# noce2/FluidFramework

Hardware: AMD Instinct MI355X
Metric: sequenced merge-tree ops applied/sec (node) at 100k docs; bit-exact text+props (higher is better)
Workload: dtype int32; 1 GPU; c3: 100000 docs/GPU x 10000 sequenced ops, 8 writers, refSeq lag <= 64, insert 0.5 / remove 0.3 / annotate 0.2; docs_total=100000, docs_per_gpu=100000, ops_per_doc=10000, parallelism=doc-shard x1

## Files before the change

fluidframework_amd/__init__.py:

```python
import ctypes

import numpy as np

from . import _native
from .wire import CHECKSUM_DTYPE, OP_DTYPE, Batch, Interner

__all__ = ["MergeTreeBatch", "DeviceBatch", "Batch", "Interner", "DeltaLogOverflow"]


class DeltaLogOverflow(RuntimeError):

    def __init__(self, msg, records):
        super().__init__(msg)
        self.records = records


class PinnedArray:

    def __init__(self, lib, n, dtype):
        dt = np.dtype(dtype)
        nbytes = max(int(n), 1) * dt.itemsize
        self.lib = lib
        self.p = lib.mt_host_alloc(nbytes)
        if not self.p:
# ... 347 lines not shown
        if not b:
            raise RuntimeError(f"mt_generate failed: {self.lib.mt_last_error(self.h).decode()}")
        return DeviceBatch(self, None, handle=b)

    def generated_seeds(self, cfg, doc_base=0, doc_ids=None):
        c = _native.gen_cfg(cfg)
        ids = None if doc_ids is None else np.ascontiguousarray(doc_ids, dtype=np.int32)
        off = np.zeros(self.n_docs + 1, dtype=np.int64)
        self._check(self.lib.mt_generated_seeds_docs(self.h, ctypes.byref(c), doc_base, _native.ptr(ids),
                                                     _native.ptr(off), None), "mt_generated_seeds")
        seed = np.zeros(max(int(off[-1]), 1), dtype=np.uint16)
        self._check(self.lib.mt_generated_seeds_docs(self.h, ctypes.byref(c), doc_base, _native.ptr(ids),
                                                     _native.ptr(off), _native.ptr(seed)), "mt_generated_seeds")
        return off, seed

    def sync(self):
        self._check(self.lib.mt_sync(self.h), "mt_sync")

    def last_hbm_docs(self):
        out = np.zeros(8, dtype=np.uint32)
        self._check(self.lib.mt_last_hbm_docs(self.h, _native.ptr(out)), "mt_last_hbm_docs")
        return dict(total=int(out[0]), spilled=int(out[1]), segments=int(out[2]), blocks=int(out[3]), heap=int(out[4]),
                    text=int(out[5]), props=int(out[6]), at_load=int(out[7]))

    def last_paged_peaks(self):
        out = np.zeros(5, dtype=np.uint32)
        self._check(self.lib.mt_last_paged_peaks(self.h, _native.ptr(out)), "mt_last_paged_peaks")
        return dict(pages=int(out[0]), unsettled=int(out[1]), heap=int(out[2]), segments=int(out[3]),
                    tight_handovers=int(out[4]))

    def last_zamboni(self):
        out = np.zeros(2, dtype=np.uint32)
        self._check(self.lib.mt_last_zamboni(self.h, _native.ptr(out)), "mt_last_zamboni")
        return {"in_place": int(out[0]), "fallback": int(out[1])}

    def last_grown(self):
        out = np.zeros(6, dtype=np.uint32)
        self._check(self.lib.mt_last_grown(self.h, _native.ptr(out)), "mt_last_grown")
        return dict(zip(["grown", "rounds", "in_big_region", "pages", "unsettled", "heap"], (int(x) for x in out)))

    def last_kernel_ms(self):
        return float(self.lib.mt_last_kernel_ms(self.h))

    def set_stream_priority(self, priority):
        self._check(self.lib.mt_set_stream_priority(self.h, int(priority)), "mt_set_stream_priority")

    def last_load_ms(self):
        return float(self.lib.mt_last_load_ms(self.h))

    def status(self):
        out = np.zeros(self.n_docs, dtype=np.int32)
        self._check(self.lib.mt_get_status(self.h, _native.ptr(out)), "mt_get_status")
        return out

    def get_length(self, doc):
        out = ctypes.c_uint32()
        self._check(self.lib.mt_get_length(self.h, doc, ctypes.byref(out)), "mt_get_length")
        return out.value

    def get_text(self, doc):
        n = ctypes.c_uint32()
        self._check(self.lib.mt_get_text(self.h, doc, None, 0, ctypes.byref(n)), "mt_get_text")
        buf = np.zeros(max(n.value, 1), dtype=np.uint16)
        self._check(self.lib.mt_get_text(self.h, doc, _native.ptr(buf), n.value, ctypes.byref(n)),
                    "mt_get_text")
        return buf[: n.value].tobytes().decode("utf-16-le", errors="surrogatepass")

# ... 282 lines not shown
```

fluidframework_amd/_native.py:

```python
import ctypes
import os

import numpy as np

from .wire import CHECKSUM_DTYPE, OP_DTYPE

HERE = os.path.dirname(os.path.abspath(__file__))
MT_E_INVALID, MT_E_HIP, MT_E_NOMEM, MT_E_NODEVICE, MT_E_OVERFLOW, MT_E_STALE_VIEW = -1, -2, -3, -4, -5, -6
LIB_PATH = os.environ.get("MT_LIB_PATH") or os.path.join(HERE, "libmtreplay.so")


class MtOptions(ctypes.Structure):
    _fields_ = [("device", ctypes.c_int32), ("seg_capacity", ctypes.c_int32),
                ("block_capacity", ctypes.c_int32), ("heap_capacity", ctypes.c_int32),
                ("text_capacity", ctypes.c_int32), ("props_capacity", ctypes.c_int32),
                ("delta_log_capacity", ctypes.c_int32), ("lds_seg_capacity", ctypes.c_int32),
                ("page_capacity", ctypes.c_int32), ("page_heap_capacity", ctypes.c_int32),
                ("unsettled_capacity", ctypes.c_int32), ("uid_capacity", ctypes.c_int32),
                ("lds_page_capacity", ctypes.c_int32), ("lds_unsettled_capacity", ctypes.c_int32),
                ("lds_page_heap_capacity", ctypes.c_int32), ("lds_narrow_overlap", ctypes.c_int32),
                ("delta_log_mode", ctypes.c_int32), ("live_client", ctypes.c_int32),
                ("live_group_capacity", ctypes.c_int32), ("paged_slices", ctypes.c_int32),
                ("segment_ordinals", ctypes.c_int32), ("overlap_arena_capacity", ctypes.c_int32)]

# ... 19 lines not shown
                ("p_newline", ctypes.c_uint64), ("p_len_continue", ctypes.c_uint64),
                ("p_insert_props", ctypes.c_uint64), ("p_null", ctypes.c_uint64)]


_P, _I, _U32, _U64 = ctypes.c_void_p, ctypes.c_int, ctypes.c_uint32, ctypes.c_uint64
SIGNATURES = [
    ("mt_create", _P, [_U32, _P]),
    ("mt_destroy", None, [_P]),
    ("mt_last_error", ctypes.c_char_p, [_P]),
    ("mt_num_docs", _U32, [_P]),
    ("mt_load_initial_text", _I, [_P, _P, _P]),
    ("mt_start_collaboration", _I, [_P, _P, _P]),
    ("mt_reset", _I, [_P]),
    ("mt_apply_ops", _I, [_P, _P, _P, _U64, _P, _U64, _P, _U64]),
    ("mt_load_snapshots", _I, [_P, _P, _P, _P, _U64, _P, _U64, _P, _U64, _P, _P]),
    ("mt_extract_snapshots", _I, [_P, _P, _P, _P, _P, _P, _P]),
    ("mt_snapshots_upload", _P, [_P, _P, _P, _P, _U64, _P, _U64, _P, _U64, _P, _P]),
    ("mt_snapshots_upload_range", _P, [_P, _U32, _U32, _P, _P, _P, _U64, _P, _U64, _P, _U64, _P, _P]),
    ("mt_snapshots_load_async", _I, [_P, _P]),
    ("mt_snapshots_free", None, [_P]),
    ("mt_batch_upload", _P, [_P, _P, _P, _U64, _P, _U64, _P, _U64]),
    ("mt_batch_apply_async", _I, [_P, _P]),
    ("mt_batch_num_ops", _U64, [_P]),
    ("mt_batch_free", None, [_P]),
    ("mt_host_alloc", ctypes.c_void_p, [ctypes.c_uint64]),
    ("mt_host_free", None, [ctypes.c_void_p]),
    ("mt_sync", _I, [_P]),
    ("mt_last_kernel_ms", ctypes.c_float, [_P]),
    ("mt_set_stream_priority", ctypes.c_int, [_P, ctypes.c_int]),
    ("mt_last_load_ms", ctypes.c_float, [_P]),
    ("mt_last_hbm_docs", _I, [_P, _P]),
    ("mt_last_paged_peaks", _I, [_P, _P]),
    ("mt_last_zamboni", _I, [_P, _P]),
    ("mt_last_grown", _I, [_P, _P]),
    ("mt_generate", _P, [_P, _P, _U32, _P]),
    ("mt_generate_docs", _P, [_P, _P, _U32, _P, _P, _P]),
    ("mt_generated_seeds_docs", _I, [_P, _P, _U32, _P, _P, _P]),
    ("mt_generated_seeds", _I, [_P, _P, _U32, _P, _P]),
    ("mt_batch_sizes", _I, [_P, _P, _P, _P]),
    ("mt_batch_download", _I, [_P, _P, _P, _P, _P]),
    ("mt_get_status", _I, [_P, _P]),
    ("mt_get_length", _I, [_P, _U32, _P]),
    ("mt_get_text", _I, [_P, _U32, _P, _U32, _P]),
    ("mt_get_texts", _I, [_P, _U32, _P, _P, _P, ctypes.c_uint16, _P, _P, _U64]),
    ("mt_get_texts_device", _I, [_P, _U32, _P, _P, _P, ctypes.c_uint16, _P, _P, _U64]),
    ("mt_last_text_ms", _I, [_P, _P]),
    ("mt_get_prop_runs", _I, [_P, _U32, _P, _U32, _P, _P, _U32, _P]),
    ("mt_get_segments", _I, [_P, _U32, _P, _U32, _P, _P, _U32, _P]),
    ("mt_get_segment_props", _I, [_P, _U32, _U32, _P, _U32, _P]),
    ("mt_get_all_segment_props", _I, [_P, _U32, _P, ctypes.c_uint64, _P]),
    ("mt_get_overlap_arena", _I, [_P, _U32, _P]),
    ("mt_get_delta_log", _I, [_P, _U32, _P, _U32, _P]),
    ("mt_delta_log_reset", _I, [_P]),
    ("mt_debug_raw", _I, [_P, _U32, _P, _U32, _P, _P]),
    ("mt_debug_prof", _I, [_P, _P, _I]),
    ("mt_maintenance_counts", _I, [_P, _P]),
    ("mt_checksums", _I, [_P, _P]),
    ("mt_checksums_device", _I, [_P, _P]),
    ("mt_regenerate_pending", _I, [_P, _U32, _P, _U32, _P, _P, _U32, _P, _U32]),
    ("mt_pending_counts", _I, [_P, _P]),
    ("mt_debug_heap", _I, [_P, _U32, _P, _U32, _P, _P, _U32, _P]),
    ("mt_get_containing_segment", _I, [_P, _U32, ctypes.c_int32, ctypes.c_int32, ctypes.c_int32, _P, _P, _U32]),
    ("mt_get_segment_by_uid", _I, [_P, _U32, _U32, ctypes.c_int32, ctypes.c_int32, _P, _P, _U32]),
    ("mt_get_view_lengths", _I, [_P, _U32, _P, _P, _P, _P]),
]

# ... 31 lines not shown
```

fluidframework_amd/csrc/mt_engine.h:

```cpp
#pragma once
#include <type_traits>

#include "mt_device.h"

#define LDS_AS __attribute__((address_space(3)))
#define GLB_AS __attribute__((address_space(1)))

template <bool kLogT> struct TierLdsT {
    static constexpr bool kLds = true;
    static constexpr bool kLog = kLogT;
    static constexpr bool kPaged = false;
    static constexpr bool kLive = false;
    static constexpr int kOvlBits = 32;
    static constexpr bool kMayGrow = false;
    static constexpr bool kOvf = false;
    typedef uint32_t O_v;
    typedef LDS_AS v4i *A_t;
    typedef LDS_AS uint32_t *O_t;
    typedef LDS_AS v4u *B_t;
    typedef LDS_AS v2i *H_t;
};
template <bool kLogT> struct TierGlbT {
    static constexpr bool kLds = false;
    static constexpr bool kLog = kLogT;
// ... 742 lines not shown
        wsync<T>();
        if (!has_parent) {
            const int nl = d.depth;
            if (nl >= MT_LV) {
                fail_cap(d, 2);
                return;
            }
            d.depth++;
            if (lane() == 0) {
                d.nb[nl] = 1;
                lvl(d, nl)[0] = 2;
            }
            wsync<T>();
            if (ordon(d)) ord_canon_all(d);
            return;
        }
        const int pc = cntr(d, l + 1, P) + 1;
        wsync<T>();
        if (lane() == 0) lvl(d, l + 1)[P] = (uint8_t)pc;
        wsync<T>();
        if (pc < MT_MAXN) {
            if (ordon(d)) {
                ord_put(ordl(d, l) + b + 1, uni((int)ordl(d, l)[b]) + ord_w(pc));
                ord_canon(d, l, b);
                ord_canon(d, l, b + 1);
            }
            return;
        }
        l = l + 1;
        b = P;
    }
}

TD void blk_replace(DocT<T> &d, int l, int b0, int nold, int k, int base, int extra) {
    if (nbr(d, l) + (k - nold) > bcap(d, l)) {
        fail_cap(d, 2);
        return;
    }
    blk_shift(d, l, b0 + nold, k - nold);
    LDS_AS uint8_t *c = lvl(d, l);
    for (int j = lane(); j < k; j += MT_WAVE) {
        c[b0 + j] = (uint8_t)(base + (j < extra ? 1 : 0));
        if (l == 0) d.flg[b0 + j] = MT_SCOUR_UNDEF;
    }
    wsync<T>();
}

TD void compute_ends(DocT<T> &d) {
    const LDS_AS uint8_t *c = lvl(d, 0);
    const int nb = nbr(d, 0);
    int carry = 0;
    for (int base = 0; base < nb; base += MT_WAVE) {
        const int b = base + lane();
        const int v = b < nb ? c[b] : 0;
        const int inc = wave_scan_incl(v);
        if (b < nb) d.ends[b] = (uint16_t)(carry + inc);
        carry += bcast(inc, MT_WAVE - 1);
    }
    wsync<T>();
}
TD int block_of(DocT<T> &d, int i, int nb) {
    int lo = 0, hi = nb - 1;
    while (lo < hi) {
        const int mid = (lo + hi) >> 1;
        if (d.ends[mid] > i)
            hi = mid;
// ... 1065 lines not shown
        }
        wsync<T>();
    }
    return keep;
}

#ifdef MT_PROF
TD void pack_impl(DocT<T> &d, int l, int b);
TD void pack(DocT<T> &d, int l, int b) {
    PROF_WRAP_BEGIN
    pack_impl(d, l, b);
    PROF_WRAP_END(3)
    
}
TD void pack_impl(DocT<T> &d, int l, int b) {
#else
TD void pack(DocT<T> &d, int l, int b) {
#endif
    while (true) {
        int c0;
        const int P = blk_find(d, l + 1, b, true, c0);
        if (P < 0) {
            FAIL_INTERNAL(d);
            return;
        }
        const int nch = cntr(d, l + 1, P);
        int total = 0;
        if (l == 0) {
            total = scour_range(d, blk_prefix(d, 0, c0), c0, nch);
            if (d.status) return;
        } else {
            for (int cb = c0; cb < c0 + nch; cb++) total += cntr(d, l, cb);
        }
        int k = total / MT_HALF;
        if (k > MT_MAXN - 1) k = MT_MAXN - 1;
        if (k < 1) k = 1;
        const int base = total / k, extra = total % k;
        blk_replace(d, l, c0, nch, k, base, extra);
        if (d.status) return;
        if (lane() == 0) lvl(d, l + 1)[P] = (uint8_t)k;
        wsync<T>();
        if (k < MT_HALF && l + 2 < d.depth) {
            l = l + 1;
            b = P;
            continue;
        }
        if (ordon(d)) ord_canon(d, l + 1, P);
        return;
    }
}

TD void pack_counts(DocT<T> &d, int l, int b, int &top_l, int &top_b) {
    while (true) {
        int c0;
        const int P = blk_find(d, l + 1, b, true, c0);
        if (P < 0) {
            FAIL_INTERNAL(d);
            return;
        }
        const int nch = cntr(d, l + 1, P);
        int total = 0;
        for (int cb = c0; cb < c0 + nch; cb++) total += cntr(d, l, cb);
        int k = total / MT_HALF;
        if (k > MT_MAXN - 1) k = MT_MAXN - 1;
        if (k < 1) k = 1;
        blk_replace(d, l, c0, nch, k, total / k, total % k);
        if (d.status) return;
        if (lane() == 0) lvl(d, l + 1)[P] = (uint8_t)k;
        wsync<T>();
        if (k < MT_HALF && l + 2 < d.depth) {
            l = l + 1;
            b = P;
            continue;
        }
        top_l = l + 1;
        top_b = P;
        return;
    }
}

#ifdef MT_PROF
TD void zamboni_impl(DocT<T> &d);
TD void zamboni(DocT<T> &d) {
    PROF_WRAP_BEGIN
    zamboni_impl(d);
    PROF_WRAP_END(4)
    
}
TD void zamboni_impl(DocT<T> &d) {
#else
TD void zamboni(DocT<T> &d) {
#endif
    for (int it = 0; it < MT_ZAMBONI && d.status == 0; it++) {
        if (d.heap_n == 0) break;
        const v2i top = heap_top(d);
        if (top.x > d.min_seq) break;
        heap_pop(d);
        wsync<T>();
        P2_T0(12)
// ... 879 lines not shown
```

fluidframework_amd/csrc/mt_kernels.h:

```cpp
#pragma once
#include "../../include/mt_replay.h"
#include "mt_paged.h"

__device__ static void init_doc_hdr(const DevState &st, int doc, int len) {
    DocHdr h;
    memset(&h, 0, sizeof(h));
    h.depth = 1;
    h.n_blk[0] = 1;
    h.text_top = len;
    h.props_top = 1;
    h.next_uid = 2;
    h.delta_hash = MT_FNV_OFF;
    h.status = len > st.T ? MT_DOC_CAPACITY : 0;
    const size_t S = st.S;
    if (len > 0) {
        h.n_seg = 1;
        st.segA[doc * S] = v4i{len, 0, MT_RSEQ_NONE, pack_cli(-1, 0)};
        st.segO[doc * S] = 0ull;
        st.segB[doc * S] = v4u{0u, 0u, 1u, 0u};
        if (st.segP) {
            u64 *w = (u64 *)(st.segP + doc * S);
            w[0] = w[1] = w[2] = w[3] = 0ull;
        }
    }
// ... 378 lines not shown
            q[0] = len;
            q[1] = d.n;
            q[2] = r;
            q[3] = c;
        }
        OpIn in;
        gen_op(g, cfg, t, r, c, msn, len, in, ops_out, text_out, props_out, doc);
        apply_op(d, in, gt, gp);
    }
    gen_end(g, used_out, doc);
    if (T::kLds && d.status == MT_DOC_RETRY) {
        if (lane() == 0) st.retry[doc] = 1;
        return;
    }
    if (lane() == 0) {
        if (d.status) fail_out[doc] = d.status;
        if (!T::kLds) st.retry[doc] = 0;
    }
    store_doc(d, st, doc);
}

template <class T>
__device__ __forceinline__ void pg_peaks(const DevState &st, PagedDoc<T> &pd, int pk_ut, int pk_heap) {
    const int np = nbr(pd.up, 1);
    int ns = 0;
    for (int q = lane(); q < np; q += MT_WAVE) ns += pm_nseg(pd, pd.up.dir[q]);
    ns = wave_sum(ns);
    if (lane() == 0) {
        atomicMax(st.stats + 8, (uint32_t)np);
        atomicMax(st.stats + 9, (uint32_t)pk_ut);
        atomicMax(st.stats + 10, (uint32_t)pk_heap);
        atomicMax(st.stats + 11, (uint32_t)ns);
        if constexpr (pg_zinplace<T>()) {
            const uint32_t zi = pg_zcount(pd)[0], zf = pg_zcount(pd)[1];
            if (zi) atomicAdd(st.stats + 16, zi);
            if (zf) atomicAdd(st.stats + 17, zf);
        }
    }
}
#ifndef MT_PAGED_WAVES
#define MT_PAGED_WAVES 3
#endif
#ifndef MT_HM_WAVES
#define MT_HM_WAVES 2
#endif
#ifndef MT_FULL_WAVES
#define MT_FULL_WAVES 2
#endif
#ifndef MT_PACKED_WAVES
#define MT_PACKED_WAVES 2
#endif
template <class T> constexpr int paged_waves() {
    return T::kHM ? MT_HM_WAVES
                  : (T::kMayGrow ? MT_FULL_WAVES : (T::kPacked ? MT_PACKED_WAVES : MT_PAGED_WAVES));
}
#if MT_PAGED_WAVES > 0
#define MT_PAGED_WPE __attribute__((amdgpu_waves_per_eu(paged_waves<T>())))
#else
#define MT_PAGED_WPE
#endif
template <class T>
__device__ __forceinline__ void pg_handover(const DevState &st, int doc, int64_t k, const PagedCaps &pc) {
    if (lane() == 0) {
        st.retry[doc] = pc.tight ? 2 : 3;
        st.resume[doc] = k;
        atomicAdd(st.stats + (pc.tight ? 12 : 13), 1u);
    }
}
struct PagedSlice {
// ... 240 lines not shown
```

fluidframework_amd/csrc/mt_paged.h:

```cpp
#pragma once
#include "mt_engine.h"

#ifdef MT_PROF
#define PG_T0(k) const unsigned long long _pt##k = __builtin_amdgcn_s_memtime();
#define PG_T1(k)                                                         \
    if (lane() == 0) {                                                   \
        pd.w.prof[k] += __builtin_amdgcn_s_memtime() - _pt##k;           \
        pd.w.prof[64 + k] += 1ull;                                       \
    }
#define PG_CNT(k)                                                        \
    if (lane() == 0) pd.w.prof[64 + k] += 1ull;
#else
#define PG_T0(k)
#define PG_T1(k)
#define PG_CNT(k)
#endif

template <class T> struct PagedDoc {
    DocT<T> w;
    DocT<T> up;
    LDS_AS PageMeta *meta;
    GLB_AS PageMeta *gmeta;
    LDS_AS int *pvl;
    LDS_AS int *cob;
// ... 33 lines not shown
    LDS_AS int *sob;
    int sob_ch;
    int wnb, wobs;
};

struct PagedCaps {
    int PP, PH, UT;
    int tight;
    int stage;
    int narrow;
    int grow;
    int packed;
};

#define PW_B 16
#define MT_PK_MASKS 256

struct PagedLayout {
    uint32_t offWA, offWB, offWO, offWcnt, offWflg, offWends, offWscr, offWnb;
    uint32_t offUcnt, offUnb, offDir, offMeta, offCob, offHeap, offUpage, offUA, offUO, offGen, offProf,
        total;
};
static __host__ __device__ inline PagedLayout paged_layout(int PP, int PH, int UT, int gen_words, int ob,
                                                           bool packed = false, bool hm = false) {
    PagedLayout L;
    uint32_t o = 0;
    L.offWA = o; o += 16u * MT_PG_SLOTS;
    L.offWB = o; o += 16u * MT_PG_SLOTS;
    L.offWO = o; o += (uint32_t)ob * MT_PG_SLOTS;
    L.offUA = o; o += (packed ? 12u : 16u) * UT;
    o = (o + 7u) & ~7u;
    L.offUO = o; o += packed ? 8u * MT_PK_MASKS + MT_PK_MASKS / 8 : ((((uint32_t)ob * UT) + 7u) & ~7u);
    L.offHeap = o; o += 8u * (PH + 1);
    L.offMeta = o; o += hm ? 0u : (uint32_t)sizeof(PageMeta) * PP + 8u;
    L.offUpage = o; o += packed ? 0u : (2u * UT + 3u) & ~3u;
    L.offCob = o; o += hm ? 8u * (uint32_t)((PP + 63) / 64) + 4u * 64 : 4u * PP;
    L.offWscr = o; o += 64u * 4;
    L.offWnb = o; o += MT_LV * 4;
    L.offUnb = o; o += MT_LV * 4;
    L.offGen = o; o += 4u * gen_words;
    L.offDir = o; o += 2u * PP;
    L.offWends = o; o += 2u * PW_B;
    L.offWcnt = o; o += (uint32_t)MT_LV * PW_B;
    L.offWflg = o; o += PW_B;
    L.offUcnt = o; o += (uint32_t)(pcnt_bytes(PP) - PP);
#ifdef MT_PROF
    o = (o + 7u) & ~7u;
    L.offProf = o; o += 128u * 8;
#else
    L.offProf = 0;
#endif
    L.total = (o + 15u) & ~15u;
    return L;
}

TD PagedDoc<T> &pdoc(DocT<T> &w) { return *reinterpret_cast<PagedDoc<T> *>(&w); }
template <class T> __device__ __forceinline__ PagedCaps eff_caps(PagedCaps pc) {
    if constexpr (T::kPP > 0) pc.PP = T::kPP;
    if constexpr (T::kPH > 0) pc.PH = T::kPH;
    if constexpr (T::kUT > 0) pc.UT = T::kUT;
    return pc;
}
TD void pg_fail_cap(DocT<T> &w, int cause) {
    if (w.status == 0) w.cap_cause = cause;
    fail(w, MT_DOC_CAPACITY);
}
__device__ __forceinline__ PageMeta pm_load(const LDS_AS PageMeta *m) {
// ... 981 lines not shown
        asm volatile("" ::"v"(touch));
#else
        pg_win_switch(pd, pg);
#endif
    }
    pd.cur_pos = pos;
    pd.w.obs_base = obs_base;
}

TD void pg_pack1_impl(PagedDoc<T> &pd, int pos);
TD void pg_pack1(PagedDoc<T> &pd, int pos) {
    PG_T0(14)
    pg_pack1_impl(pd, pos);
    PG_T1(14)
}
TD void pg_pack1_impl(PagedDoc<T> &pd, int pos) {
    DocT<T> &w = pd.w;
    DocT<T> &up = pd.up;
    pg_win_flush(pd);
    pd.cur = -1;
    pd.zuid = 0;
    int c0;
    const int P = blk_find(up, 2, pos, true, c0);
    if (P < 0) {
        FAIL_INTERNAL(w);
        return;
    }
    const int nch = cntr(up, 2, P);
    int TB = 0, TS = 0;
    for (int j = 0; j < nch; j++) {
        TB += cntr(up, 1, c0 + j);
        TS += uni(pm_nseg(pd, up.dir[c0 + j]));
    }
    int k = TB / MT_HALF;
    if (k > MT_MAXN - 1) k = MT_MAXN - 1;
    if (k < 1) k = 1;
    const int base = TB / k, extra = TB % k;
    if (nbr(up, 1) + k > pd.PP) {
        pg_fail_cap(w, 7);
        return;
    }
    if constexpr (T::kHM) {
        gsync();
        gsync_rd();
    }
    const int bl = lane();
    int opg = -1, ob = 0, bseg0 = 0;
    uint32_t obc = 0, of2 = 0;
    {
        int acc_b = 0, acc_s = 0;
        for (int j = 0; j < nch; j++) {
            const int pg = uni(up.dir[c0 + j]);
            const int nb = uni(pm_nblk(pd, pg));
            if (bl >= acc_b && bl < acc_b + nb) {
                opg = pg;
                ob = bl - acc_b;
                pm_blocks(pd, pg, obc, of2);
                int s = acc_s;
                for (int q = 0; q < ob; q++) s += pm_bc_of(obc, q);
                bseg0 = s;
            }
            acc_b += nb;
            acc_s += uni(pm_nseg(pd, pg));
        }
    }
    const int bcnt = opg >= 0 ? pm_bc_of(obc, ob) : 0;
    const int8_t bflg = opg >= 0 ? pm_fl_of(of2, ob) : (int8_t)0;
    auto nb0 = [&](int m) { return m * base + min(m, extra); };
    LDS_AS int32_t *newp = w.scr;
    for (int m = 0; m < k; m++) {
// ... 64 lines not shown
    for (int j = 0; j < nch; j++) {
        const int pg = uni(up.dir[c0 + j]);
        if (lane() == 0) pm_set_ns(pd, pg, 0, 0);
        wsync<T>();
    }
    blk_replace(up, 1, c0, nch, k, base, extra);
    if (up.status) {
        pg_fail_cap(w, 7);
        return;
    }
    for (int m = 0; m < k; m++)
        if (lane() == 0) up.dir[c0 + m] = (uint16_t)newp[m];
    if (lane() == 0) lvl(up, 2)[P] = (uint8_t)k;
    wsync<T>();
    pg_cob_rebuild(pd);
    int top_l = 2, top_b = P;
    if (k < MT_HALF && 3 < up.depth) pack_counts(up, 2, P, top_l, top_b);
    if (up.status) {
        if (w.status == 0) w.cap_cause = up.cap_cause;
        fail(w, MT_DOC_INTERNAL);
        return;
    }
    if (ordon(w)) ord_canon(up, top_l, top_b);
}

TD LDS_AS uint32_t *pg_zcount(PagedDoc<T> &pd) { return (LDS_AS uint32_t *)(pd.meta + pd.PP); }
template <class T> constexpr bool pg_zinplace() {
#ifdef MT_NO_ZINPLACE
    return false;
#else
    return !T::kLog && !T::kHM && !T::kLive;
#endif
}
TD bool pg_scour_inplace(PagedDoc<T> &pd, int pg, uint32_t uid) {
    DocT<T> &w = pd.w;
    const int k = lane();
    const int n = uni(pm_nseg(pd, pg)), nb = uni(pm_nblk(pd, pg));
    v4i a = v4i{0, 0, 0, 0};
    v4u b = v4u{0, 0, 0, 0};
    if (k < n) {
        a = pd.gA[(size_t)pg * MT_PG_SLOTS + k];
        b = pd.gB[(size_t)pg * MT_PG_SLOTS + k];
    }
    uint32_t bc, f2;
    pm_blocks(pd, pg, bc, f2);
    bc = (uint32_t)uni((int)bc);
    f2 = (uint32_t)uni((int)f2);
    const u64 hit = ballot(k < n && (b.z & ~MT_MARKER_BIT) == uid);
    if (!hit) {
        PG_CNT(19)
        return false;
    }
    const int i = first_lane(hit);
    int q = 0, bstart = 0;
    while (q < nb && q < 8 && i >= bstart + pm_bc_of(bc, q)) {
        bstart += pm_bc_of(bc, q);
        q++;
    }
    if (q >= nb || q >= 8) {
        FAIL_INTERNAL(w);
        return false;
    }
    if (pm_fl_of(f2, q) == 0) {
        PG_CNT(20)
        return false;
    }
    const int cnt = pm_bc_of(bc, q);
    if (pd.up.depth < 2 || bstart + cnt > n) return true;
    const bool in = k >= bstart && k < bstart + cnt;
    bool nl_res;
    const ScourPlan pl = scour_plan(w, a, b, in, false, bstart, nl_res);
    const int keep = __popcll(pl.m_surv);
    if (pl.big || (keep < cnt && keep < MT_HALF)) return true;
    const ScourGroups g = scour_groups(a, in, pl.m_join, pl.m_surv);
    if (g.m_grp && w.text_top + g.totc > w.T_cap) return true;
    PG_CNT(21)
    PG_CNT(37)
    if (k == 0) pg_zcount(pd)[0]++;
    const uint32_t nbc = (bc & ~(15u << (4 * q))) | ((uint32_t)keep << (4 * q));
    const uint32_t nf2 = (f2 & ~(3u << (2 * q))) | (1u << (2 * q));
    if (g.m_grp) {
        gsync_rd();
        scour_merge(w, a, b, in, g);
    }
    if (keep < cnt || g.m_grp) {
        const u64 blk = ((1ull << cnt) - 1ull) << bstart;
        const u64 chg = g.m_grp | (blk & ~pl.m_surv);
        const int first = __ffsll((long long)chg) - 1;
        const bool surv = (pl.m_surv >> k) & 1ull;
        const int dst = in ? bstart + __popcll(pl.m_surv & ((1ull << k) - 1ull)) : k - (cnt - keep);
        const bool st = k < n && k >= first && (in ? surv : keep < cnt);
        const bool mv = st && dst != k;
        u64 o = 0;
        if (mv) o = pd.gO[(size_t)pg * MT_PG_SLOTS + k];
        asm volatile("" : "+v"(o));
        if (st) {
            pd.gA[(size_t)pg * MT_PG_SLOTS + dst] = a;
            pd.gB[(size_t)pg * MT_PG_SLOTS + dst] = b;
        }
        if (mv) pd.gO[(size_t)pg * MT_PG_SLOTS + dst] = o;
    } else {
        PG_CNT(38)
    }
    if (k == 0) {
        pd.meta[pg].bc = nbc;
        pd.meta[pg].flg2 = (uint16_t)nf2;
// ... 863 lines not shown
        pd.gmeta = (GLB_AS PageMeta *)tier_paged<T::kBig>(st, doc).meta;
        pd.sob = pd.cdl + (pc.PP + 63) / 64;
        pd.sob_ch = -1;
        pd.wnb = pd.wobs = 0;
    } else {
        pd.meta = (LDS_AS PageMeta *)(smem + L.offMeta);
    }
    pd.vgen = 0;
    pd.scr_ch = -1;
    pd.upage = (LDS_AS uint16_t *)(smem + L.offUpage);
    pd.uA = (LDS_AS v4i *)(smem + L.offUA);
    pd.uO = (LDS_AS typename T::O_v *)(smem + L.offUO);
    if constexpr (T::kPacked) {
        pd.uL = (LDS_AS uint32_t *)(smem + L.offUA);
        pd.uS = pd.uL + pc.UT;
        pd.uP = pd.uS + pc.UT;
        pd.sbase = h.cur_seq - 32000;
        pd.uM = (LDS_AS u64 *)(smem + L.offUO);
        pd.mbm = (LDS_AS uint32_t *)(smem + L.offUO + 8u * MT_PK_MASKS);
        if (lane() < MT_PK_MASKS / 32) pd.mbm[lane()] = lane() == 0 ? 1u : 0u;
        if (lane() == 0) pd.uM[0] = 0;
    }
    pd.cur = -1;
    pd.cur_pos = -1;
    pd.dirty = 0;
    pd.tdirty = 0;
    pd.vvalid = 0;
    pd.wgrow = 0;
    pd.opbound = 0;
    pd.zuid = 0;
    pd.zpv = 0;
    pd.press = 0;
    if constexpr (!T::kHM) {
        if (lane() == 0) pg_zcount(pd)[0] = pg_zcount(pd)[1] = 0;
    }
    pd.ovf_top = MT_OVF_HDR;
    pd.ovf_last = 0;
    pd.ovf_maxn = 0;
    pd.ovf_half = 0;
    pd.ovf_made = 0;
    pd.ovf_peak = 0;
    if constexpr (T::kOvf) {
        if (pd.govf) {
            const GLB_AS uint32_t *hw = (const GLB_AS uint32_t *)pd.govf;
            pd.ovf_top = max((int)hw[0], MT_OVF_HDR);
            pd.ovf_last = (int)hw[1];
            pd.ovf_maxn = (int)hw[2];
            pd.ovf_made = hw[4];
            pd.ovf_peak = (int)hw[5];
            pd.ovf_half = ((int)hw[3] & 1) && pd.ovf_top > mt_ovf_mid(pd.OA) ? 1 : 0;
        }
    }
}

TD void pg_mark_free(PagedDoc<T> &pd) {
    const int np = nbr(pd.up, 1);
    pd.vvalid = 0;
    for (int base = 0; base < pd.PP; base += MT_WAVE)
        if (base + lane() < pd.PP) pm_set_nblk(pd, base + lane(), pm_nblk(pd, base + lane()) | 0x80);
    wsync<T>();
    for (int base = 0; base < np; base += MT_WAVE)
        if (base + lane() < np) {
            const int pg = pd.up.dir[base + lane()];
            pm_set_nblk(pd, pg, pm_nblk(pd, pg) & 0x7F);
        }
    wsync<T>();
    for (int base = 0; base < pd.PP; base += MT_WAVE) {
// ... 291 lines not shown
```

fluidframework_amd/csrc/mt_replay.hip:

```cpp
#include <hip/hip_runtime.h>

#include <algorithm>
#include <cstdlib>
#include <cstdio>
#include <cstring>
#include <string>
#include <vector>

#include "../../include/mt_replay.h"
#include "mt_kernels.h"
#include "mt_variants.h"
#ifdef MT_SINGLE_TU
#define MT_VARIANT_DEF(n, k) const void *mtk_##n() { return (const void *)k; }
MT_VARIANTS(MT_VARIANT_DEF)
#endif

__global__ void __launch_bounds__(MT_WAVE) k_init(DevState st, const int64_t *seed_off,
                                                  const uint16_t *seed) {
    const int doc = blockIdx.x;
    if (doc >= st.n_docs) return;
    oslot_reset(st, doc);
    if (st.bslot && lane() == 0) st.bslot[doc] = -1;
    const int64_t s0 = seed_off ? seed_off[doc] : 0, s1 = seed_off ? seed_off[doc + 1] : 0;
    const int len = (int)(s1 - s0);
// ... 1834 lines not shown
    return 0;
}

int mt_last_grown(mt_handle *h, uint32_t *out) {
    if (!h || !out) return MT_E_INVALID;
    SETTLE(h);
    uint32_t in_big = 0;
    for (int32_t x : h->bslot_h) in_big += x >= 0;
    out[0] = h->grown_last;
    out[1] = h->grow_rounds_last;
    out[2] = in_big;
    out[3] = (uint32_t)h->big_caps.PP;
    out[4] = (uint32_t)h->big_caps.UT;
    out[5] = (uint32_t)h->big_caps.PH;
    return 0;
}

int mt_last_paged_peaks(mt_handle *h, uint32_t *out) {
    if (!h || !out) return MT_E_INVALID;
    HIPCHK(h, hipSetDevice(h->device));
    SETTLE(h);
    HIPCHK(h, hipMemcpy(out, h->st.stats + 8, 5 * sizeof(uint32_t), hipMemcpyDeviceToHost));
    return 0;
}

int mt_last_zamboni(mt_handle *h, uint32_t *out) {
    if (!h || !out) return MT_E_INVALID;
    HIPCHK(h, hipSetDevice(h->device));
    SETTLE(h);
    HIPCHK(h, hipMemcpy(out, h->st.stats + 16, 2 * sizeof(uint32_t), hipMemcpyDeviceToHost));
    return 0;
}

int mt_apply_ops(mt_handle *h, const int64_t *doc_op_off, const mt_op_rec *ops, uint64_t n_ops,
                 const uint16_t *text, uint64_t text_len, const uint32_t *props,
                 uint64_t props_len) {
    if (!h) return MT_E_INVALID;
    h->err.clear();
    mt_batch *b = mt_batch_upload(h, doc_op_off, ops, n_ops, text, text_len, props, props_len);
    if (!b) return h->err.rfind("mt_batch_upload: device", 0) == 0 ? MT_E_NOMEM : MT_E_INVALID;
    int rc = mt_batch_apply_async(h, b);
    if (rc == 0) rc = mt_sync(h);
    mt_batch_free(b);
    return rc;
}

struct mt_snapshots {
    int device = 0;
    uint32_t doc_lo = 0, n_docs = 0;
    int64_t *off = nullptr;
    int32_t *nh = nullptr, *min_seq = nullptr, *cur_seq = nullptr;
    mt_seg_rec *segs = nullptr;
    uint16_t *text = nullptr;
    uint32_t *props = nullptr;
    mt_batch *body = nullptr;
    LoadScratch sc = {nullptr, nullptr, nullptr, nullptr, nullptr, nullptr};
    int64_t *sc_off = nullptr;
    bool any_big = false;
};

void mt_snapshots_free(mt_snapshots *s) {
    if (!s) return;
    hipSetDevice(s->device);
    void *ps[] = {s->off, s->nh, s->min_seq, s->cur_seq, s->segs, s->text, s->props, s->sc.A, s->sc.O, s->sc.B,
                  s->sc.cnt, s->sc.flg, s->sc_off};
    for (void *p : ps)
// ... 1351 lines not shown
```

include/mt_replay.h:

```cpp
#ifndef MT_REPLAY_H
#define MT_REPLAY_H
#include <stddef.h>
#include <stdint.h>

#include "mt_types.h"

#ifdef __cplusplus
extern "C" {
#endif

#define MT_E_INVALID (-1)
#define MT_E_HIP (-2)
#define MT_E_NOMEM (-3)
#define MT_E_NODEVICE (-4)
#define MT_E_OVERFLOW (-5)
#define MT_E_STALE_VIEW (-6)

typedef struct mt_handle mt_handle;
typedef struct mt_batch mt_batch;

typedef struct mt_options {
    int32_t device;
    int32_t seg_capacity;
    int32_t block_capacity;
// ... 41 lines not shown
int mt_load_snapshots(mt_handle *h, const int64_t *doc_seg_off, const int32_t *n_header, const mt_seg_rec *segs,
                      uint64_t n_segs, const uint16_t *text, uint64_t text_len, const uint32_t *props,
                      uint64_t props_len, const int32_t *min_seq, const int32_t *cur_seq);
typedef struct mt_snapshots mt_snapshots;
mt_snapshots *mt_snapshots_upload(mt_handle *h, const int64_t *doc_seg_off, const int32_t *n_header,
                                  const mt_seg_rec *segs, uint64_t n_segs, const uint16_t *text, uint64_t text_len,
                                  const uint32_t *props, uint64_t props_len, const int32_t *min_seq,
                                  const int32_t *cur_seq);
mt_snapshots *mt_snapshots_upload_range(mt_handle *h, uint32_t doc_lo, uint32_t n_docs, const int64_t *doc_seg_off,
                                        const int32_t *n_header, const mt_seg_rec *segs, uint64_t n_segs,
                                        const uint16_t *text, uint64_t text_len, const uint32_t *props,
                                        uint64_t props_len, const int32_t *min_seq, const int32_t *cur_seq);
int mt_snapshots_load_async(mt_handle *h, const mt_snapshots *s);
void mt_snapshots_free(mt_snapshots *s);
float mt_last_load_ms(mt_handle *h);

int mt_extract_snapshots(mt_handle *h, int64_t *io, mt_seg_rec *recs, uint16_t *text, uint32_t *props,
                         int32_t *min_seq, int32_t *cur_seq);

mt_batch *mt_batch_upload(mt_handle *h, const int64_t *doc_op_off, const mt_op_rec *ops,
                          uint64_t n_ops, const uint16_t *text, uint64_t text_len,
                          const uint32_t *props, uint64_t props_len);
int mt_batch_apply_async(mt_handle *h, const mt_batch *b);
uint64_t mt_batch_num_ops(const mt_batch *b);
void mt_batch_free(mt_batch *b);
void *mt_host_alloc(uint64_t bytes);
void mt_host_free(void *p);
int mt_sync(mt_handle *h);
float mt_last_kernel_ms(const mt_handle *h);
int mt_set_stream_priority(mt_handle *h, int priority);
int mt_last_hbm_docs(mt_handle *h, uint32_t *out);
int mt_last_paged_peaks(mt_handle *h, uint32_t *out);
int mt_last_zamboni(mt_handle *h, uint32_t *out);

int mt_last_grown(mt_handle *h, uint32_t *out);

mt_batch *mt_generate(mt_handle *h, const mt_gen_cfg *cfg, uint32_t doc_index_base,
                      int32_t *view_len_trace );
mt_batch *mt_generate_docs(mt_handle *h, const mt_gen_cfg *cfg, uint32_t doc_index_base,
                           const int32_t *ops_per_doc, const int32_t *doc_ids, int32_t *view_len_trace);
int mt_generated_seeds_docs(mt_handle *h, const mt_gen_cfg *cfg, uint32_t doc_index_base, const int32_t *doc_ids,
                            int64_t *seed_off, uint16_t *seed_text);
int mt_generated_seeds(mt_handle *h, const mt_gen_cfg *cfg, uint32_t doc_index_base,
                       int64_t *seed_off, uint16_t *seed_text);
int mt_batch_sizes(const mt_batch *b, uint64_t *n_ops, uint64_t *text_len, uint64_t *props_len);
int mt_batch_download(const mt_batch *b, int64_t *doc_op_off, mt_op_rec *ops, uint16_t *text,
                      uint32_t *props);

int mt_get_status(mt_handle *h, int32_t *out_status);
int mt_get_length(mt_handle *h, uint32_t doc, uint32_t *out);
int mt_get_text(mt_handle *h, uint32_t doc, uint16_t *out, uint32_t cap, uint32_t *out_len);
int mt_get_texts(mt_handle *h, uint32_t n, const uint32_t *docs, const int32_t *start,
                 const int32_t *end, uint16_t marker_unit, int64_t *off, uint16_t *out, uint64_t cap);
int mt_get_texts_device(mt_handle *h, uint32_t n, const uint32_t *docs, const int32_t *start,
                        const int32_t *end, uint16_t marker_unit, void *off_dev, void *out_dev, uint64_t cap);
int mt_last_text_ms(mt_handle *h, float *out );
int mt_get_prop_runs(mt_handle *h, uint32_t doc, uint32_t *runs, uint32_t cap_runs,
                     uint32_t *n_runs, uint32_t *records, uint32_t cap_words,
                     uint32_t *n_words);
int mt_get_segments(mt_handle *h, uint32_t doc, int32_t *rows, uint32_t cap_rows,
                    uint32_t *n_rows, int32_t *leaves, uint32_t cap_leaves, uint32_t *n_leaves);
int mt_get_overlap_arena(mt_handle *h, uint32_t doc, int32_t *out );
int mt_get_all_segment_props(mt_handle *h, uint32_t doc, int32_t *out, uint64_t cap_words, uint64_t *n_words);
int mt_get_segment_props(mt_handle *h, uint32_t doc, uint32_t seg_index, uint32_t *pairs,
                         uint32_t cap_pairs, int32_t *n_pairs);
typedef struct mt_seg_info {
// ... 50 lines not shown
```

Baseline: 162.3 million ops/s.

## Pack underfull pages in place during zamboni scour instead of falling back

When an in-place scour on a page would leave fewer than half-full blocks, a new path re-plans the surviving segments with lane permutes, merges groups twice, rewrites the page slots and block counts, and updates the parent level. Previously this case returned to the slower fallback zamboni path. A counter for in-place packs is added with a host query. This adds substantial divergent wave logic and extra metadata, and carries correctness risk for bit-exact output.

```diff
diff --git a/fluidframework_amd/__init__.py b/fluidframework_amd/__init__.py
--- a/fluidframework_amd/__init__.py
+++ b/fluidframework_amd/__init__.py
@@ -403,7 +403,9 @@
     def last_zamboni(self):
         out = np.zeros(2, dtype=np.uint32)
         self._check(self.lib.mt_last_zamboni(self.h, _native.ptr(out)), "mt_last_zamboni")
-        return {"in_place": int(out[0]), "fallback": int(out[1])}
+        packs = np.zeros(1, dtype=np.uint32)
+        self._check(self.lib.mt_last_zamboni_packs(self.h, _native.ptr(packs)), "mt_last_zamboni_packs")
+        return {"in_place": int(out[0]), "fallback": int(out[1]), "in_place_packs": int(packs[0])}
 
     def last_grown(self):
         out = np.zeros(6, dtype=np.uint32)
diff --git a/fluidframework_amd/_native.py b/fluidframework_amd/_native.py
--- a/fluidframework_amd/_native.py
+++ b/fluidframework_amd/_native.py
@@ -75,6 +75,7 @@
     ("mt_last_hbm_docs", _I, [_P, _P]),
     ("mt_last_paged_peaks", _I, [_P, _P]),
     ("mt_last_zamboni", _I, [_P, _P]),
+    ("mt_last_zamboni_packs", _I, [_P, _P]),
     ("mt_last_grown", _I, [_P, _P]),
     ("mt_generate", _P, [_P, _P, _U32, _P]),
     ("mt_generate_docs", _P, [_P, _P, _U32, _P, _P, _P]),
diff --git a/fluidframework_amd/csrc/mt_engine.h b/fluidframework_amd/csrc/mt_engine.h
--- a/fluidframework_amd/csrc/mt_engine.h
+++ b/fluidframework_amd/csrc/mt_engine.h
@@ -798,6 +798,15 @@
     }
 }
 
+struct PackSplit {
+    int k, base, extra;
+};
+__device__ __forceinline__ PackSplit pack_split(int total) {
+    int k = total / MT_HALF;
+    if (k > MT_MAXN - 1) k = MT_MAXN - 1;
+    if (k < 1) k = 1;
+    return PackSplit{k, total / k, total % k};
+}
 TD void blk_replace(DocT<T> &d, int l, int b0, int nold, int k, int base, int extra) {
     if (nbr(d, l) + (k - nold) > bcap(d, l)) {
         fail_cap(d, 2);
@@ -1929,11 +1938,9 @@
         } else {
             for (int cb = c0; cb < c0 + nch; cb++) total += cntr(d, l, cb);
         }
-        int k = total / MT_HALF;
-        if (k > MT_MAXN - 1) k = MT_MAXN - 1;
-        if (k < 1) k = 1;
-        const int base = total / k, extra = total % k;
-        blk_replace(d, l, c0, nch, k, base, extra);
+        const PackSplit ps = pack_split(total);
+        const int k = ps.k;
+        blk_replace(d, l, c0, nch, k, ps.base, ps.extra);
         if (d.status) return;
         if (lane() == 0) lvl(d, l + 1)[P] = (uint8_t)k;
         wsync<T>();
@@ -1958,10 +1965,9 @@
         const int nch = cntr(d, l + 1, P);
         int total = 0;
         for (int cb = c0; cb < c0 + nch; cb++) total += cntr(d, l, cb);
-        int k = total / MT_HALF;
-        if (k > MT_MAXN - 1) k = MT_MAXN - 1;
-        if (k < 1) k = 1;
-        blk_replace(d, l, c0, nch, k, total / k, total % k);
+        const PackSplit ps = pack_split(total);
+        const int k = ps.k;
+        blk_replace(d, l, c0, nch, k, ps.base, ps.extra);
         if (d.status) return;
         if (lane() == 0) lvl(d, l + 1)[P] = (uint8_t)k;
         wsync<T>();
diff --git a/fluidframework_amd/csrc/mt_kernels.h b/fluidframework_amd/csrc/mt_kernels.h
--- a/fluidframework_amd/csrc/mt_kernels.h
+++ b/fluidframework_amd/csrc/mt_kernels.h
@@ -434,9 +434,10 @@
         atomicMax(st.stats + 10, (uint32_t)pk_heap);
         atomicMax(st.stats + 11, (uint32_t)ns);
         if constexpr (pg_zinplace<T>()) {
-            const uint32_t zi = pg_zcount(pd)[0], zf = pg_zcount(pd)[1];
+            const uint32_t zi = pg_zcount(pd)[0], zf = pg_zcount(pd)[1], zp = pg_zcount(pd)[2];
             if (zi) atomicAdd(st.stats + 16, zi);
             if (zf) atomicAdd(st.stats + 17, zf);
+            if (zp) atomicAdd(st.stats + 18, zp);
         }
     }
 }
diff --git a/fluidframework_amd/csrc/mt_paged.h b/fluidframework_amd/csrc/mt_paged.h
--- a/fluidframework_amd/csrc/mt_paged.h
+++ b/fluidframework_amd/csrc/mt_paged.h
@@ -89,7 +89,7 @@
     o = (o + 7u) & ~7u;
     L.offUO = o; o += packed ? 8u * MT_PK_MASKS + MT_PK_MASKS / 8 : ((((uint32_t)ob * UT) + 7u) & ~7u);
     L.offHeap = o; o += 8u * (PH + 1);
-    L.offMeta = o; o += hm ? 0u : (uint32_t)sizeof(PageMeta) * PP + 8u;
+    L.offMeta = o; o += hm ? 0u : (uint32_t)sizeof(PageMeta) * PP + 12u;
     L.offUpage = o; o += packed ? 0u : (2u * UT + 3u) & ~3u;
     L.offCob = o; o += hm ? 8u * (uint32_t)((PP + 63) / 64) + 4u * 64 : 4u * PP;
     L.offWscr = o; o += 64u * 4;
@@ -1137,10 +1137,8 @@
         TB += cntr(up, 1, c0 + j);
         TS += uni(pm_nseg(pd, up.dir[c0 + j]));
     }
-    int k = TB / MT_HALF;
-    if (k > MT_MAXN - 1) k = MT_MAXN - 1;
-    if (k < 1) k = 1;
-    const int base = TB / k, extra = TB % k;
+    const PackSplit ps = pack_split(TB);
+    const int k = ps.k, base = ps.base, extra = ps.extra;
     if (nbr(up, 1) + k > pd.PP) {
         pg_fail_cap(w, 7);
         return;
@@ -1271,6 +1269,112 @@
     return !T::kLog && !T::kHM && !T::kLive;
 #endif
 }
+template <class T> constexpr bool pg_zpack() {
+#ifdef MT_NO_ZPACK
+    return false;
+#else
+    return pg_zinplace<T>();
+#endif
+}
+__device__ __forceinline__ int lane_push(int v, int dst) { return __builtin_amdgcn_ds_permute(dst << 2, v); }
+TD bool pg_pack_inplace(PagedDoc<T> &pd, int pg, v4i a, v4u b, const ScourPlan &pl, uint32_t bc, int q, int bstart) {
+    DocT<T> &w = pd.w;
+    const int k = lane();
+    const int n = uni(pm_nseg(pd, pg)), nb = uni(pm_nblk(pd, pg));
+    const int cnt = pm_bc_of(bc, q);
+    const int keep = __popcll(pl.m_surv);
+    const int n1 = n - (cnt - keep);
+    if (nb > 8) return true;
+    const bool in = k >= bstart && k < bstart + cnt;
+    const u64 below = (1ull << k) - 1ull;
+    const ScourGroups g1 = scour_groups(a, in, pl.m_join, pl.m_surv);
+    v4i a1 = a;
+    v4u b1 = b;
+    if (g1.m_grp) {
+        const uint32_t lastw = (uint32_t)__shfl((int)b.w, g1.gend & (MT_WAVE - 1), MT_WAVE);
+        if ((g1.m_grp >> k) & 1ull) {
+            a1.x = g1.glen;
+            b1.w = lastw & (SEGF_NL_KNOWN | SEGF_NL);
+        }
+    }
+    const int d1 = k < bstart ? k
+                   : !in      ? k - (cnt - keep)
+                   : ((pl.m_surv >> k) & 1ull) ? bstart + __popcll(pl.m_surv & below) : MT_WAVE - 1;
+    a1 = v4i{lane_push(a1.x, d1), lane_push(a1.y, d1), lane_push(a1.z, d1), lane_push(a1.w, d1)};
+    b1 = v4u{(uint32_t)lane_push((int)b1.x, d1), (uint32_t)lane_push((int)b1.y, d1),
+             (uint32_t)lane_push((int)b1.z, d1), (uint32_t)lane_push((int)b1.w, d1)};
+    const int src1 = lane_push(k, d1);
+    const bool in2 = k < n1;
+    int start2 = 0;
+    {
+        int st = 0;
+        for (int j = 0; j < nb; j++) {
+            if (k >= st) start2 = st;
+            st += j == q ? keep : pm_bc_of(bc, j);
+        }
+    }
+    bool nl2;
+    const ScourPlan p2 = scour_plan(w, a1, b1, in2, false, start2, nl2);
+    if (p2.big) return true;
+    const int total = __popcll(p2.m_surv);
+    const PackSplit ps = pack_split(total);
+    if (ps.k < MT_HALF && pd.up.depth > 2) return true;
+    const ScourGroups g2 = scour_groups(a1, in2, p2.m_join, p2.m_surv);
+    if ((g1.m_grp | g2.m_grp) && w.text_top + g1.totc + g2.totc > w.T_cap) return true;
+    int pos = -1;
+    if (ps.k != nb) {
+        pos = pg_pos(pd, pg);
+        if (pos < 0) return true;
+    }
+    PG_CNT(21)
+    PG_CNT(37)
+    PG_CNT(39)
+    if (k == 0) {
+        pg_zcount(pd)[0]++;
+        pg_zcount(pd)[2]++;
+    }
+    if (g1.m_grp) {
+        gsync_rd();
+        scour_merge(w, a, b, in, g1);
+        const uint32_t x1 = (uint32_t)lane_push((int)b.x, d1), w1 = (uint32_t)lane_push((int)b.w, d1);
+        if (in2 && ((g1.m_grp >> src1) & 1ull)) {
+            b1.x = x1;
+            b1.w = w1;
+        }
+    }
+    if (g2.m_grp) {
+        gsync_rd();
+        scour_merge(w, a1, b1, in2, g2);
+    }
+    {
+        const u64 chg1 = g1.m_grp | ((((1ull << cnt) - 1ull) << bstart) & ~pl.m_surv);
+        const u64 chg2 = g2.m_grp | (((1ull << n1) - 1ull) & ~p2.m_surv);
+        int first = __ffsll((long long)chg1) - 1;
+        if (chg2) first = min(first, __ffsll((long long)chg2) - 1);
+        const int dst = __popcll(p2.m_surv & below);
+        const bool st = in2 && ((p2.m_surv >> k) & 1ull) && k >= first;
+        const bool mv = st && dst != src1;
+        u64 o = 0;
+        if (mv) o = pd.gO[(size_t)pg * MT_PG_SLOTS + src1];
+        asm volatile("" : "+v"(o));
+        if (st) {
+            pd.gA[(size_t)pg * MT_PG_SLOTS + dst] = a1;
+            pd.gB[(size_t)pg * MT_PG_SLOTS + dst] = b1;
+        }
+        if (mv) pd.gO[(size_t)pg * MT_PG_SLOTS + dst] = o;
+    }
+    if (k == 0) {
+        uint32_t nbc = 0;
+        for (int j = 0; j < ps.k; j++) nbc |= (uint32_t)(ps.base + (j < ps.extra ? 1 : 0)) << (4 * j);
+        pd.meta[pg].bc = nbc;
+        pd.meta[pg].flg2 = 0;
+        pm_set_ns(pd, pg, total, ps.k);
+        if (pos >= 0) lvl(pd.up, 1)[pos] = (uint8_t)ps.k;
+    }
+    wsync<T>();
+    return false;
+}
+
 TD bool pg_scour_inplace(PagedDoc<T> &pd, int pg, uint32_t uid) {
     DocT<T> &w = pd.w;
     const int k = lane();
@@ -1310,7 +1414,11 @@
     bool nl_res;
     const ScourPlan pl = scour_plan(w, a, b, in, false, bstart, nl_res);
     const int keep = __popcll(pl.m_surv);
-    if (pl.big || (keep < cnt && keep < MT_HALF)) return true;
+    if (pl.big) return true;
+    if (keep < cnt && keep < MT_HALF) {
+        if constexpr (pg_zpack<T>()) return pg_pack_inplace(pd, pg, a, b, pl, bc, q, bstart);
+        return true;
+    }
     const ScourGroups g = scour_groups(a, in, pl.m_join, pl.m_surv);
     if (g.m_grp && w.text_top + g.totc > w.T_cap) return true;
     PG_CNT(21)
@@ -2240,7 +2348,7 @@
     pd.zpv = 0;
     pd.press = 0;
     if constexpr (!T::kHM) {
-        if (lane() == 0) pg_zcount(pd)[0] = pg_zcount(pd)[1] = 0;
+        if (lane() == 0) pg_zcount(pd)[0] = pg_zcount(pd)[1] = pg_zcount(pd)[2] = 0;
     }
     pd.ovf_top = MT_OVF_HDR;
     pd.ovf_last = 0;
diff --git a/fluidframework_amd/csrc/mt_replay.hip b/fluidframework_amd/csrc/mt_replay.hip
--- a/fluidframework_amd/csrc/mt_replay.hip
+++ b/fluidframework_amd/csrc/mt_replay.hip
@@ -1890,6 +1890,14 @@
     return 0;
 }
 
+int mt_last_zamboni_packs(mt_handle *h, uint32_t *out) {
+    if (!h || !out) return MT_E_INVALID;
+    HIPCHK(h, hipSetDevice(h->device));
+    SETTLE(h);
+    HIPCHK(h, hipMemcpy(out, h->st.stats + 18, sizeof(uint32_t), hipMemcpyDeviceToHost));
+    return 0;
+}
+
 int mt_apply_ops(mt_handle *h, const int64_t *doc_op_off, const mt_op_rec *ops, uint64_t n_ops,
                  const uint16_t *text, uint64_t text_len, const uint32_t *props,
                  uint64_t props_len) {
diff --git a/include/mt_replay.h b/include/mt_replay.h
--- a/include/mt_replay.h
+++ b/include/mt_replay.h
@@ -97,6 +97,7 @@
 int mt_last_hbm_docs(mt_handle *h, uint32_t *out);
 int mt_last_paged_peaks(mt_handle *h, uint32_t *out);
 int mt_last_zamboni(mt_handle *h, uint32_t *out);
+int mt_last_zamboni_packs(mt_handle *h, uint32_t *out);
 
 int mt_last_grown(mt_handle *h, uint32_t *out);
 
```

After: 166.1 million ops/s (median of 6 runs). +2.4%, better.
